# turian/inverse-audio-synthesis

Hardware: AMD Instinct MI355X
Metric: audio-seconds rendered+lossed/sec (whole node), batch=128 4s@44.1kHz (higher is better)
Workload: dtype f32; 1 GPU; BASELINE configs[1]: torchsynth-style Voice render + PQMF(3) analysis + mel-L1 loss, batch 128 x 4 s @ 44100 Hz per GPU; batch_per_gpu=128, samples_per_voice=176400, launch=hipgraph, streams=5, pipelined=True

## Files before the change

inverse-audio-synthesis_amd/csrc/spectral_kernels.hip:

```cpp
#include "ias_common.h"
#include <cstdlib>

#define SP_WAVES_MAX 12
static int stft_waves(int n_fft) {
  static const int env = ias_diag_env("IAS_STFT_WAVES") ? atoi(ias_diag_env("IAS_STFT_WAVES")) : 0;
  if (n_fft == 1024) return (env == 8 || env == 10) ? env : 4;
  if (n_fft == 2048) return env == 4 ? 4 : 12;
  return 4;
}

typedef float cpx __attribute__((ext_vector_type(2)));
typedef float f32x4 __attribute__((ext_vector_type(4)));
__host__ __device__ static inline int mel_padded_words(int mel_nnz, int n_out) {
  return n_out > 0 ? ((mel_nnz + 3 * n_out + 3) & ~3) : 0;
}
__device__ __forceinline__ cpx cmk(float x, float y) { return (cpx){x, y}; }
__device__ __forceinline__ cpx cadd(cpx a, cpx b) { return a + b; }
__device__ __forceinline__ cpx csub(cpx a, cpx b) { return a - b; }
#ifdef IAS_DIAG
__device__ __forceinline__ cpx cmul(cpx a, cpx b) {
  return __builtin_elementwise_fma((cpx){-a.y, a.y}, (cpx){b.y, b.x}, (cpx){a.x, a.x} * b);
}
__device__ __forceinline__ cpx cmul_negi(cpx a) { return (cpx){a.y, -a.x}; }
__device__ __forceinline__ cpx cadd_negi(cpx a, cpx x) { return a + cmul_negi(x); }
__device__ __forceinline__ cpx csub_negi(cpx a, cpx x) { return a - cmul_negi(x); }
__device__ __forceinline__ cpx cnegi_sub(cpx x, cpx a) { return cmul_negi(x) - a; }
#else
__device__ __forceinline__ cpx cmul(cpx a, cpx b) {
  return cmk(__builtin_fmaf(-a.y, b.y, a.x * b.x), __builtin_fmaf(a.y, b.x, a.x * b.y));
}
__device__ __forceinline__ cpx cadd_negi(cpx a, cpx x) {
  cpx r; asm("v_pk_add_f32 %0, %1, %2 op_sel:[0,1] op_sel_hi:[1,0] neg_hi:[0,1]" : "=v"(r) : "v"(a), "v"(x)); return r;
}
__device__ __forceinline__ cpx csub_negi(cpx a, cpx x) {
  cpx r; asm("v_pk_add_f32 %0, %1, %2 op_sel:[0,1] op_sel_hi:[1,0] neg_lo:[0,1]" : "=v"(r) : "v"(a), "v"(x)); return r;
}
__device__ __forceinline__ cpx cnegi_sub(cpx x, cpx a) {
  cpx r; asm("v_pk_add_f32 %0, %1, %2 op_sel:[1,0] op_sel_hi:[0,1] neg_lo:[0,1] neg_hi:[1,1]" : "=v"(r) : "v"(x), "v"(a)); return r;
}
#endif

__device__ __forceinline__ void dft4(cpx& v0, cpx& v1, cpx& v2, cpx& v3) {
  const cpx t0 = cadd(v0, v2), t1 = csub(v0, v2), t2 = cadd(v1, v3), t3 = csub(v1, v3);
  v0 = cadd(t0, t2); v1 = cadd_negi(t1, t3); v2 = csub(t0, t2); v3 = csub_negi(t1, t3);
}
__device__ __forceinline__ void dft8(cpx* v) {
  cpx e0 = v[0], e1 = v[2], e2 = v[4], e3 = v[6];
  cpx o0 = v[1], o1 = v[3], o2 = v[5], o3 = v[7];
  dft4(e0, e1, e2, e3);
  dft4(o0, o1, o2, o3);
  const float h = 0.70710678118654752f;
  o1 = cadd_negi(o1, o1) * h;
  o3 = cnegi_sub(o3, o3) * h;
  v[0] = cadd(e0, o0); v[4] = csub(e0, o0);
  v[1] = cadd(e1, o1); v[5] = csub(e1, o1);
  v[2] = cadd_negi(e2, o2); v[6] = csub_negi(e2, o2);
  v[3] = cadd(e3, o3); v[7] = csub(e3, o3);
}
__device__ __forceinline__ void dft16(cpx* v) {
  cpx e[8], o[8];
#pragma unroll
  for (int i = 0; i < 8; ++i) { e[i] = v[2 * i]; o[i] = v[2 * i + 1]; }
  dft8(e);
  dft8(o);
  const float c1 = 0.92387953251128674f, s1 = 0.38268343236508977f, h = 0.70710678118654752f;
  const cpx w[8] = {cmk(1.f, 0.f), cmk(c1, -s1), cmk(h, -h), cmk(s1, -c1),
                    cmk(0.f, -1.f), cmk(-s1, -c1), cmk(-h, -h), cmk(-c1, -s1)};
#pragma unroll
  for (int k = 0; k < 8; ++k) {
    const cpx t = cmul(o[k], w[k]);
    v[k] = cadd(e[k], t);
    v[k + 8] = csub(e[k], t);
  }
}
template <int R> __device__ __forceinline__ void dftR(cpx* v);
template <> __device__ __forceinline__ void dftR<4>(cpx* v) { dft4(v[0], v[1], v[2], v[3]); }
template <> __device__ __forceinline__ void dftR<8>(cpx* v) { dft8(v); }
template <> __device__ __forceinline__ void dftR<16>(cpx* v) { dft16(v); }

__device__ __forceinline__ int reflect_index(int i, int T) {
  if (i < 0) i = -i;
  if (i >= T) i = 2 * (T - 1) - i;
  return i;
}

__device__ __forceinline__ float wave_sum_f(float v) {
#pragma unroll
  for (int d = 32; d > 0; d >>= 1) v += __shfl_xor(v, d, 64);
  return v;
}

struct SpecArgs {
  const float* audio;
  const float* tables;
  const int* mel_start;
  const int* mel_count;
  const int* mel_woff;
  const float* mel_w;
  float* out;
  const float* target;
  double* partials;
  const float* rowpeak;
  int T, F, hop, n_out, mel_nnz;
  int groups;
  int value_mode;
  int loss_mode;
  float eps;
};

__device__ __forceinline__ void wave_lds_sync() {
#ifdef IAS_STFT_DRAIN_SYNC
  asm volatile("s_waitcnt lgkmcnt(0)" ::: "memory");
  __builtin_amdgcn_wave_barrier();
#else
  __builtin_amdgcn_fence(__ATOMIC_RELEASE, "wavefront");
  __builtin_amdgcn_wave_barrier();
  __builtin_amdgcn_fence(__ATOMIC_ACQUIRE, "wavefront");
#endif
}

typedef unsigned x_u2 __attribute__((ext_vector_type(2)));
template <int L> __device__ __forceinline__ void xchg_pair(float& f0, float& f1) {
  unsigned r0 = __float_as_uint(f0), r1 = __float_as_uint(f1);
  if (L == 5) { const x_u2 t = __builtin_amdgcn_permlane32_swap(r0, r1, false, false); r0 = t.x; r1 = t.y; }
  else if (L == 4) { const x_u2 t = __builtin_amdgcn_permlane16_swap(r0, r1, false, false); r0 = t.x; r1 = t.y; }
  else {
    const unsigned old0 = r0;
    r0 = __builtin_amdgcn_update_dpp(r0, r1, 0x128 , 0xf, 0xc, false);
    r1 = __builtin_amdgcn_update_dpp(r1, old0, 0x128, 0xf, 0x3, false);
  }
  f0 = __uint_as_float(r0); f1 = __uint_as_float(r1);
}
__device__ __forceinline__ void xchg_reg_lane345(cpx (&u)[8]) {
#pragma unroll
  for (int comp = 0; comp < 2; ++comp) {
    float f[8];
#pragma unroll
    for (int q = 0; q < 8; ++q) f[q] = comp ? u[q].y : u[q].x;
    xchg_pair<3>(f[0], f[1]); xchg_pair<3>(f[2], f[3]); xchg_pair<3>(f[4], f[5]); xchg_pair<3>(f[6], f[7]);
    xchg_pair<4>(f[0], f[2]); xchg_pair<4>(f[1], f[3]); xchg_pair<4>(f[4], f[6]); xchg_pair<4>(f[5], f[7]);
    xchg_pair<5>(f[0], f[4]); xchg_pair<5>(f[1], f[5]); xchg_pair<5>(f[2], f[6]); xchg_pair<5>(f[3], f[7]);
#pragma unroll
    for (int q = 0; q < 8; ++q) { if (comp) u[q].y = f[q]; else u[q].x = f[q]; }
  }
}
#ifndef IAS_S2_REGX
#define IAS_S2_REGX 1
#endif

template <int R, int N2>
__device__ __forceinline__ void load_frame(const float* __restrict__ arow, int T, int hop, int f, int lane,
                                           float (&x)[2 * R]) {
  const int g0 = f * hop - N2;
  if (g0 >= 0 && g0 + 2 * N2 <= T && (((g0 | T) & 1) == 0)) {
    typedef float f32x2_t __attribute__((ext_vector_type(2)));
    typedef const __attribute__((address_space(1))) f32x2_t* glb_f2p;
    glb_f2p p = (glb_f2p)(reinterpret_cast<const f32x2_t*>(arow + g0) + lane);
#ifndef IAS_LOADFRAME_PLAIN
    asm volatile("" : "+v"(p));
#endif
#pragma unroll
    for (int n1 = 0; n1 < R; ++n1) { const f32x2_t q = p[64 * n1]; x[2 * n1] = q[0]; x[2 * n1 + 1] = q[1]; }
  } else {
#pragma unroll
    for (int n1 = 0; n1 < R; ++n1) {
      const int m = g0 + 2 * (64 * n1 + lane);
      x[2 * n1] = arow[reflect_index(m, T)];
      x[2 * n1 + 1] = arow[reflect_index(m + 1, T)];
#ifndef IAS_LOADFRAME_PLAIN
      asm volatile("" : "+v"(x[2 * n1]), "+v"(x[2 * n1 + 1]));
#endif
    }
  }
}

template <int LOG2N, int SP_WAVES, bool LOSS2 >
__global__ __launch_bounds__(64 * SP_WAVES, SP_WAVES == 10 ? 5 : 1) void stft_kernel(const SpecArgs a) {
  constexpr int SP_THREADS = 64 * SP_WAVES;
  constexpr int NFFT = 1 << LOG2N, N2 = NFFT / 2, R = N2 / 64, NPAIR = 8 * R, NP_IT = (NPAIR + 63) / 64;
  constexpr int SCR = NPAIR * 9;
  constexpr int NUNP = (N2 / 2) / 64 + 1;
  extern __shared__ __attribute__((aligned(16))) float smem[];
  cpx* s_scr = reinterpret_cast<cpx*>(smem);
  float* s_melw = reinterpret_cast<float*>(s_scr + SP_WAVES * SCR);
  const int melw_words = mel_padded_words(a.mel_nnz, a.mel_start != nullptr ? a.n_out : 0);
  int* s_meli = reinterpret_cast<int*>(s_melw + melw_words);

  const int tid = threadIdx.x, lane = tid & 63, wave = tid >> 6;
  const int b = blockIdx.y;
  const float* arow = a.audio + (size_t)b * a.T;
  const bool mel = a.mel_start != nullptr;
  float pscale = 1.0f;
  if (a.rowpeak != nullptr) { const float pkv = a.rowpeak[b]; if (pkv > 1.0f) { const float r = 1.0f / pkv; pscale = r * r; } }

  if (mel) {
    for (int i = tid; i < melw_words; i += SP_THREADS) s_melw[i] = 0.0f;
    for (int i = tid; i < a.n_out; i += SP_THREADS) {
      s_meli[i] = a.mel_start[i];
      s_meli[a.n_out + i] = (a.mel_count[i] + 3) & ~3;
    }
    __syncthreads();
    for (int i = tid; i < a.n_out; i += SP_THREADS) {
      int off = 0;
      for (int m = 0; m < i; ++m) off += s_meli[a.n_out + m];
      s_meli[2 * a.n_out + i] = off;
    }
    __syncthreads();
    for (int i = tid; i < a.n_out; i += SP_THREADS) {
      const int n = a.mel_count[i], src = a.mel_woff[i], dst = s_meli[2 * a.n_out + i];
      for (int j = 0; j < n; ++j) s_melw[dst + j] = a.mel_w[src + j];
    }
  }

  constexpr int NTAB = 64 * (2 * R + 2 * R + 16 * NP_IT + 2 * NUNP);
  cpx* s_tab = reinterpret_cast<cpx*>(s_meli + ((3 * (mel ? a.n_out : 0) + 1) & ~1));
  for (int i = tid; i < NTAB / 2; i += SP_THREADS) {
    const int pp = i >> 6, l = i & 63;
    s_tab[i] = cmk(a.tables[64 * (2 * pp) + l], a.tables[64 * (2 * pp + 1) + l]);
  }
  const cpx* t_win = s_tab + lane;
  const cpx* t_tw1 = t_win + 64 * R;
  const cpx* t_tw2 = t_tw1 + 64 * R;
  const cpx* t_twu = t_tw2 + 64 * 8 * NP_IT;
  if (mel && lane < 3) reinterpret_cast<float*>(s_scr + wave * SCR)[N2 + 1 + lane] = 0.0f;
  __syncthreads();

  cpx* sA = s_scr + wave * SCR;
  float l0 = 0.f, l1 = 0.f, l2 = 0.f;
  int h_nmaxa = 0, h_nmaxb = 0;
  if (mel) {
    if (lane < a.n_out) h_nmaxa = s_meli[a.n_out + lane];
    if (lane + 64 < a.n_out) h_nmaxb = s_meli[a.n_out + lane + 64];
  }
#pragma unroll
  for (int d = 32; d > 0; d >>= 1) {
    h_nmaxa = max(h_nmaxa, __shfl_xor(h_nmaxa, d, 64));
    h_nmaxb = max(h_nmaxb, __shfl_xor(h_nmaxb, d, 64));
  }
  h_nmaxa = __builtin_amdgcn_readfirstlane(h_nmaxa);
  h_nmaxb = __builtin_amdgcn_readfirstlane(h_nmaxb);
  const int f_begin = blockIdx.x * a.groups;
  const int f_end = min(f_begin + a.groups, a.F);

  float xc[2 * R], xn[2 * R];
  int f = f_begin + wave;
  if (f < f_end) load_frame<R, N2>(arow, a.T, a.hop, f, lane, xc);

  for (; f < f_end; f += SP_WAVES) {
    const bool more = f + SP_WAVES < f_end;
    if (more) load_frame<R, N2>(arow, a.T, a.hop, f + SP_WAVES, lane, xn);

    cpx v[R];
#pragma unroll
    for (int n1 = 0; n1 < R; ++n1)
      v[n1] = cmk(xc[2 * n1], xc[2 * n1 + 1]) * t_win[64 * n1];
    dftR<R>(v);
    {
      const int c = lane & 7, aa = lane >> 3;
#pragma unroll
      for (int k1 = 0; k1 < R; ++k1)
        sA[(k1 * 8 + c) * 9 + aa] = cmul(v[k1], t_tw1[64 * k1]);
    }
    wave_lds_sync();
    cpx u[NP_IT][8];
#pragma unroll
    for (int i = 0; i < NP_IT; ++i) {
      const int p = lane + 64 * i;
      if (p < NPAIR) {
#pragma unroll
        for (int q = 0; q < 8; ++q) u[i][q] = sA[p * 9 + q];
      }
    }
    wave_lds_sync();
#pragma unroll
    for (int i = 0; i < NP_IT; ++i) {
      const int p = lane + 64 * i;
      if (p < NPAIR) {
        const int k1 = p >> 3, c = p & 7;
        dft8(u[i]);
#pragma unroll
        for (int d = 0; d < 8; ++d)
          sA[(k1 * 8 + d) * 9 + c] = cmul(u[i][d], t_tw2[64 * (8 * i + d)]);
      }
    }
    wave_lds_sync();
#pragma unroll
    for (int i = 0; i < NP_IT; ++i) {
      const int p = lane + 64 * i;
      if (p < NPAIR) {
#pragma unroll
        for (int q = 0; q < 8; ++q) u[i][q] = sA[p * 9 + q];
      }
    }
    wave_lds_sync();
#pragma unroll
    for (int i = 0; i < NP_IT; ++i) {
      const int p = lane + 64 * i;
      if (p < NPAIR) {
        const int k1 = p >> 3, d = p & 7;
        dft8(u[i]);
#pragma unroll
        for (int e = 0; e < 8; ++e) { const int k = k1 + R * d + 8 * R * e; sA[k + (k >> 3)] = u[i][e]; }
      }
    }
    wave_lds_sync();
    float pk[NUNP], pn[NUNP];
#pragma unroll
    for (int i = 0; i < NUNP; ++i) {
      const int k = lane + 64 * i;
      pk[i] = pn[i] = 0.f;
      if (k <= N2 / 2) {
        const int kn = (N2 - k) & (N2 - 1);
        const cpx zk = sA[k + (k >> 3)], zn = sA[kn + (kn >> 3)];
        const cpx ze = cmk(0.5f * (zk.x + zn.x), 0.5f * (zk.y - zn.y));
        const cpx zo = cmk(0.5f * (zk.y + zn.y), -0.5f * (zk.x - zn.x));
        const cpx t = cmul(t_twu[64 * i], zo);
        const cpx xk = cadd(ze, t);
        const cpx xq = cmk(ze.x - t.x, -(ze.y - t.y));
        float vk = xk.x * xk.x + xk.y * xk.y, vn = xq.x * xq.x + xq.y * xq.y;
        if (a.rowpeak != nullptr) { vk *= pscale; vn *= pscale; }
        if (a.value_mode == 1) { vk = __builtin_amdgcn_sqrtf(vk); vn = __builtin_amdgcn_sqrtf(vn); }
        else if (a.value_mode == 3) { vk = __builtin_amdgcn_sqrtf(fmaxf(vk, a.eps)); vn = __builtin_amdgcn_sqrtf(fmaxf(vn, a.eps)); }
        pk[i] = vk; pn[i] = vn;
      }
    }
    wave_lds_sync();
    float* P = reinterpret_cast<float*>(sA);
#pragma unroll
    for (int i = 0; i < NUNP; ++i) {
      const int k = lane + 64 * i;
      if (k <= N2 / 2) { P[k] = pk[i]; P[N2 - k] = pn[i]; }
    }
    wave_lds_sync();
    {
      const size_t row = ((size_t)b * a.F + f) * a.n_out;
      for (int m0 = 0; m0 < a.n_out; m0 += 128) {
        const int ma = m0 + lane, mb = m0 + 64 + lane;
        const bool oka = ma < a.n_out, okb = mb < a.n_out;
        float va = 0.f, vb = 0.f;
        if (mel) {
          const int sa = oka ? s_meli[ma] : 0, na = oka ? s_meli[a.n_out + ma] : 0, woa = oka ? s_meli[2 * a.n_out + ma] : 0;
          const int sb = okb ? s_meli[mb] : 0, nb = okb ? s_meli[a.n_out + mb] : 0, wob = okb ? s_meli[2 * a.n_out + mb] : 0;
          const float* wa = s_melw + woa;
          const float* wb = s_melw + wob;
          int nmaxa = h_nmaxa, nmaxb = h_nmaxb;
          if (m0 != 0) {
            nmaxa = na; nmaxb = nb;
#pragma unroll
            for (int d = 32; d > 0; d >>= 1) {
              nmaxa = max(nmaxa, __shfl_xor(nmaxa, d, 64));
              nmaxb = max(nmaxb, __shfl_xor(nmaxb, d, 64));
            }
          }
          for (int j = 0; j < nmaxa; j += 4) {
            const bool on = j < na;
            const int jj = on ? j : 0;
            const f32x4 w = *reinterpret_cast<const f32x4*>(wa + jj);
            const float* pp = P + sa + jj;
            const float p0 = pp[0], p1 = pp[1], p2 = pp[2], p3 = pp[3];
            const float t = fmaf(w[3], p3, fmaf(w[2], p2, fmaf(w[1], p1, fmaf(w[0], p0, va))));
            va = on ? t : va;
          }
          for (int j = 0; j < nmaxb; j += 4) {
            const bool on = j < nb;
            const int jj = on ? j : 0;
            const f32x4 w = *reinterpret_cast<const f32x4*>(wb + jj);
            const float* pp = P + sb + jj;
            const float p0 = pp[0], p1 = pp[1], p2 = pp[2], p3 = pp[3];
            const float t = fmaf(w[3], p3, fmaf(w[2], p2, fmaf(w[1], p1, fmaf(w[0], p0, vb))));
            vb = on ? t : vb;
          }
        } else {
          va = oka ? P[ma] : 0.f;
          vb = okb ? P[mb] : 0.f;
        }
        float ta = 0.f, tb = 0.f;
        if (a.loss_mode != 0) {
          if (oka) ta = a.target[row + ma];
          if (okb) tb = a.target[row + mb];
        }
        if (a.out != nullptr) {
          if (oka) a.out[row + ma] = va;
          if (okb) a.out[row + mb] = vb;
        }
        if (a.loss_mode == 1) {
          if (oka) l0 += fabsf(va - ta);
          if (okb) l0 += fabsf(vb - tb);
        } else if (LOSS2) {
          if (oka) { const float d = ta - va; l0 = fmaf(d, d, l0); l1 = fmaf(ta, ta, l1); l2 += fabsf(__log2f(va) - __log2f(ta)); }
          if (okb) { const float d = tb - vb; l0 = fmaf(d, d, l0); l1 = fmaf(tb, tb, l1); l2 += fabsf(__log2f(vb) - __log2f(tb)); }
        }
      }
    }
    wave_lds_sync();
    if (more) {
#pragma unroll
      for (int e = 0; e < 2 * R; ++e) xc[e] = xn[e];
    }
  }

  if (a.partials != nullptr) {
    __shared__ float s_red[SP_WAVES][4];
    l0 = wave_sum_f(l0); l1 = wave_sum_f(l1); l2 = wave_sum_f(l2) * 0.6931471805599453f;
    if (lane == 0) { s_red[wave][0] = l0; s_red[wave][1] = l1; s_red[wave][2] = l2; }
    __syncthreads();
    if (tid < 3) {
      double sacc = 0.0;
      for (int w = 0; w < SP_WAVES; ++w) sacc += (double)s_red[w][tid];
      a.partials[((size_t)blockIdx.y * gridDim.x + blockIdx.x) * 3 + tid] = sacc;
    }
  }
}

#define IAS_SEG_MAX_ROWS 17
#define IAS_SEG_HDR 16
#define IAS_SEG_STRIDE 72
#ifndef IAS_S2_ROW
#define IAS_S2_ROW 10
#endif
#define IAS_S2_AT(row, col) ((row) * IAS_S2_ROW + (col))
#define IAS_S2_UP(i) ((i) + (IAS_S2_ROW - 8) * ((i) >> 3))
static_assert(IAS_SEG_MAX_ROWS * IAS_SEG_STRIDE + 1 <= 2 * 64 * IAS_S2_ROW, "segment-major rows fit the wave's scratch");
struct Spec2Args {
  const float* audio;
  const float* tables;
  const float* segtab;
  float* out;
  const float* target;
  double* partials;
  const float* rowpeak;
  int T, F, hop, n_out, nframes;
  unsigned magicF;
  int value_mode, loss_mode;
  float eps;
#ifdef IAS_S2_STAMPS
  unsigned long long* stamps;
#endif
};
#ifdef IAS_S2_STAMPS
static unsigned long long* g_s2_stamps = nullptr;
extern "C" int ias_stft2_set_stamps(unsigned long long* p) { g_s2_stamps = p; return 0; }
#define S2_STAMP(id)                                                                                     \
  do {                                                                                                   \
    if (a.stamps != nullptr && stamp_n < 255) {                                                          \
      const unsigned long long t_ = __builtin_amdgcn_s_memtime();                                        \
      if (lane == 0) a.stamps[((size_t)blockIdx.x * SP_WAVES + wave) * 256 + 1 + stamp_n] = (t_ << 8) | (id); \
      ++stamp_n;                                                                                         \
    }                                                                                                    \
  } while (0)
#else
#define S2_STAMP(id) do {} while (0)
#endif
__device__ __forceinline__ float wave_shr1(float x, float fill) {
  return __int_as_float(__builtin_amdgcn_update_dpp(__float_as_int(fill), __float_as_int(x), 0x138, 0xf, 0xf, false));
}
__device__ __forceinline__ float wave_shl1(float x, float fill) {
  return __int_as_float(__builtin_amdgcn_update_dpp(__float_as_int(fill), __float_as_int(x), 0x130, 0xf, 0xf, false));
}

template <int NSUB> __device__ __forceinline__ void stft2_load_frame(const float* __restrict__ arow, int T, int hop, int f,
                                                                      int lane, float (&x)[16 * NSUB]) {
  if (NSUB == 1) {
    float (&x1)[16] = reinterpret_cast<float (&)[16]>(x);
    load_frame<8, 512>(arow, T, hop, f, lane, x1);
  } else {
    const int g0 = f * hop - 1024;
    if (g0 >= 0 && g0 + 2048 <= T && ((reinterpret_cast<uintptr_t>(arow + g0) & 15) == 0)) {
      const f32x4* p = reinterpret_cast<const f32x4*>(arow + g0) + lane;
#pragma unroll
      for (int n1 = 0; n1 < 8; ++n1) {
        const f32x4 q = p[64 * n1];
        x[2 * n1] = q[0]; x[2 * n1 + 1] = q[1]; x[16 + 2 * n1] = q[2]; x[16 + 2 * n1 + 1] = q[3];
      }
    } else {
#pragma unroll
      for (int n1 = 0; n1 < 8; ++n1)
#pragma unroll
        for (int c = 0; c < 4; ++c) {
          x[16 * (c >> 1) + 2 * n1 + (c & 1)] = arow[reflect_index(g0 + 256 * n1 + 4 * lane + c, T)];
        }
    }
  }
}

#ifndef IAS_STFT2_MINW
#define IAS_STFT2_MINW 5
#endif
#if IAS_S2_REGX
#define S2X_ROW 9
#define S2X_PAD 2
#else
#define S2X_ROW IAS_S2_ROW
#define S2X_PAD (IAS_S2_ROW - 8)
#endif
#define S2X_AT(row, col) ((row) * S2X_ROW + (col))
#define S2X_UP(i) ((i) + S2X_PAD * ((i) >> 3))
static_assert(64 * S2X_ROW <= 64 * IAS_S2_ROW && 256 + S2X_PAD * 32 <= 64 * IAS_S2_ROW, "stft2 scratch indexing fits the wave's scratch");
template <int SP_WAVES, bool MEL, int LOSS, int NSUB>
__global__ __launch_bounds__(64 * SP_WAVES, NSUB == 2 ? 3 * SP_WAVES / 8 : (SP_WAVES >= 8 ? (SP_WAVES == 8 ? IAS_STFT2_MINW : SP_WAVES / 2) : (3 * SP_WAVES + 3) / 4))
void stft2_kernel(const Spec2Args a) {
  static_assert(NSUB == 1 || (NSUB == 2 && !MEL), "mel filterbanks: n_fft 1024 only");
  constexpr int SP_THREADS = 64 * SP_WAVES, N2 = 512 * NSUB, R = 8, SCR = 64 * IAS_S2_ROW, NPK = 4 * NSUB, HALF = N2 / 2;
  constexpr int NTAB = 8 * NSUB + 8 + 8 + (NSUB == 2 ? 8 : 0) + NPK;
  extern __shared__ __attribute__((aligned(16))) float smem[];
  cpx* s_scr = reinterpret_cast<cpx*>(smem);
  __shared__ cpx s_tab[NTAB * 64];
  __shared__ cpx s_segw[MEL ? IAS_SEG_MAX_ROWS * 64 : 1];
  __shared__ int s_sega[MEL ? 9 * 64 : 1];
  const int tid = threadIdx.x, lane = tid & 63;
  const int wave = __builtin_amdgcn_readfirstlane(tid >> 6);

  constexpr int OLD_UNP = 10, V2_BASE_2048 = 32 + 32 + 32 + 18;
  for (int i = tid; i < NTAB * 64; i += SP_THREADS) {
    const int pp = i >> 6, l = i & 63;
    const int src = NSUB == 2 ? V2_BASE_2048 + 2 * pp : (pp < 24 ? 2 * pp : 48 + OLD_UNP + 2 * (pp - 24));
    s_tab[i] = cmk(a.tables[64 * src + l], a.tables[64 * (src + 1) + l]);
  }
  for (int i = tid; i < SP_WAVES * SCR; i += SP_THREADS) s_scr[i] = cmk(0.f, 0.f);
  int seg_rows = 0, seg_r[3] = {0, 0, 0}, seg_s0 = 0;
  if (MEL) {
    const int* hdr = reinterpret_cast<const int*>(a.segtab);
    seg_rows = hdr[1]; seg_r[0] = hdr[2]; seg_r[1] = hdr[3]; seg_r[2] = hdr[4]; seg_s0 = hdr[5];
    for (int i = tid; i < 9 * 64; i += SP_THREADS) s_sega[i] = hdr[IAS_SEG_HDR + i];
    const cpx* wsrc = reinterpret_cast<const cpx*>(a.segtab + IAS_SEG_HDR + 9 * 64);
    for (int i = tid; i < seg_rows * 64; i += SP_THREADS) s_segw[i] = wsrc[i];
  }
  const cpx* t_win = s_tab + lane;
  const cpx* t_tw1 = t_win + 64 * 8 * NSUB;
  const cpx* t_tw2 = t_tw1 + 64 * 8;
  const cpx* t_cmb = t_tw2 + 64 * 8;
  const cpx* t_twu = t_cmb + (NSUB == 2 ? 64 * 8 : 0);
  __syncthreads();

  cpx* sA = s_scr + wave * SCR;
  float* P2 = reinterpret_cast<float*>(sA);

  float l0 = 0.f, l1 = 0.f, l2 = 0.f;
  const int gw = blockIdx.x * SP_WAVES + wave, nw = gridDim.x * SP_WAVES;
  const int k1 = lane >> 3, dd = lane & 7;

  auto row_of = [&](int fi, int& b, int& f) {
    unsigned q0 = __umulhi((unsigned)fi, a.magicF);
    int r = fi - (int)q0 * a.F;
    if (r >= a.F) { r -= a.F; ++q0; }
    b = (int)q0; f = r;
  };
  float xc[16 * NSUB], xn[16 * NSUB];
#ifdef IAS_S2_STAMPS
  int stamp_n = 0;
#endif
  int fi = gw, bcur = 0, fcur = 0;
  float pk_cur = 0.0f, pk_next = 0.0f;
  if (fi < a.nframes) {
    row_of(fi, bcur, fcur);
    stft2_load_frame<NSUB>(a.audio + (size_t)bcur * a.T, a.T, a.hop, fcur, lane, xc);
    if (a.rowpeak != nullptr) pk_cur = a.rowpeak[bcur];
#pragma unroll
    for (int e = 0; e < 16 * NSUB; ++e) asm volatile("" : "+v"(xc[e]));
    asm volatile("" : "+v"(pk_cur));
  }
  for (; fi < a.nframes; fi += nw) {
    const bool more = fi + nw < a.nframes;
    S2_STAMP(1);
    int bnext = 0, fnext = 0;
    if (more) {
      row_of(fi + nw, bnext, fnext);
      stft2_load_frame<NSUB>(a.audio + (size_t)bnext * a.T, a.T, a.hop, fnext, lane, xn);
      if (a.rowpeak != nullptr) pk_next = a.rowpeak[bnext];
    }
    float pscale = 0.25f;
    if (pk_cur > 1.0f) { const float r = __builtin_amdgcn_rcpf(pk_cur); pscale = 0.25f * (r * r); }
    const size_t row = (size_t)fi * a.n_out;
    float tgt_m[3] = {0.f, 0.f, 0.f};
    if (MEL && LOSS != 0) {
#pragma unroll
      for (int c = 0; c < 3; ++c) if (64 * c + lane < a.n_out) tgt_m[c] = a.target[row + 64 * c + lane];
    }

    const int kl = k1 + 8 * dd;
    float tg_k[NPK], tg_n[NPK], tg_mid = 0.f;
    if (!MEL && LOSS != 0) {
#pragma unroll
      for (int e = 0; e < NPK; ++e) { tg_k[e] = a.target[row + kl + 64 * e]; tg_n[e] = a.target[row + N2 - kl - 64 * e]; }
      if (lane == 0) tg_mid = a.target[row + HALF];
    }
    cpx zlo[NPK], zhi[NPK];
    cpx ue[8];
#pragma unroll
    for (int sub = 0; sub < NSUB; ++sub) {
      cpx v[R];
#pragma unroll
      for (int n1 = 0; n1 < R; ++n1) v[n1] = cmk(xc[16 * sub + 2 * n1], xc[16 * sub + 2 * n1 + 1]) * t_win[64 * (8 * sub + n1)];
      dft8(v);
      cpx u[8];
#if IAS_S2_REGX
#pragma unroll
      for (int q = 0; q < R; ++q) u[q] = cmul(v[q], t_tw1[64 * q]);
      S2_STAMP(2);
      xchg_reg_lane345(u);
      S2_STAMP(3);
      S2_STAMP(4);
#else
      {
        const int c = lane & 7, aa = lane >> 3;
#pragma unroll
        for (int q = 0; q < R; ++q) sA[S2X_AT(q * 8 + c, aa)] = cmul(v[q], t_tw1[64 * q]);
      }
      S2_STAMP(2);
      wave_lds_sync();
      S2_STAMP(3);
#pragma unroll
      for (int q = 0; q < 8; ++q) u[q] = sA[S2X_AT(lane, q)];
      wave_lds_sync();
      S2_STAMP(4);
#endif
      dft8(u);
#pragma unroll
      for (int d = 0; d < 8; ++d) sA[S2X_AT(k1 * 8 + d, dd)] = cmul(u[d], t_tw2[64 * d]);
      S2_STAMP(5);
      wave_lds_sync();
      S2_STAMP(6);
#pragma unroll
      for (int q = 0; q < 8; ++q) u[q] = sA[S2X_AT(lane, q)];
      wave_lds_sync();
      S2_STAMP(7);
      dft8(u);
      if (NSUB == 1) {
#pragma unroll
        for (int e = 0; e < 4; ++e) { zlo[e] = u[e]; zhi[e] = u[4 + e]; }
      } else if (sub == 0) {
#pragma unroll
        for (int e = 0; e < 8; ++e) ue[e] = u[e];
      } else {
#pragma unroll
        for (int e = 0; e < 8; ++e) {
          const cpx t = cmul(u[e], t_cmb[64 * e]);
          zlo[e % NPK] = cadd(ue[e], t); zhi[e % NPK] = csub(ue[e], t);
        }
      }
    }
#pragma unroll
    for (int e = 0; e < NPK; ++e) { const int i = kl + 64 * e; sA[S2X_UP(i)] = zhi[e]; }
    S2_STAMP(8);
    wave_lds_sync();
    S2_STAMP(9);
    float pk[NPK], pn[NPK];
#pragma unroll
    for (int e = 0; e < NPK; ++e) {
      const int k = kl + 64 * e;
      const int i = (HALF - k) & (HALF - 1);
      cpx zn = sA[S2X_UP(i)];
      const cpx zk = zlo[e];
      if (e == 0 && k == 0) zn = zk;
      const cpx w = t_twu[64 * e];
      const float ea = zk.x + zn.x, eb = zk.y - zn.y, od = zk.x - zn.x, os = zk.y + zn.y;
      const float tx = fmaf(w.y, od, w.x * os), ty = fmaf(-w.x, od, w.y * os);
      const float xr = ea + tx, xi = eb + ty, yr = ea - tx, yi = eb - ty;
      pk[e] = fmaf(xi, xi, xr * xr) * pscale;
      pn[e] = fmaf(yi, yi, yr * yr) * pscale;
    }
    float pmid = fmaf(zhi[0].y, zhi[0].y, zhi[0].x * zhi[0].x) * (4.0f * pscale);
    if (a.value_mode == 1) {
#pragma unroll
      for (int e = 0; e < NPK; ++e) { pk[e] = __builtin_amdgcn_sqrtf(pk[e]); pn[e] = __builtin_amdgcn_sqrtf(pn[e]); }
      pmid = __builtin_amdgcn_sqrtf(pmid);
    } else if (a.value_mode == 3) {
#pragma unroll
      for (int e = 0; e < NPK; ++e) { pk[e] = __builtin_amdgcn_sqrtf(fmaxf(pk[e], a.eps)); pn[e] = __builtin_amdgcn_sqrtf(fmaxf(pn[e], a.eps)); }
      pmid = __builtin_amdgcn_sqrtf(fmaxf(pmid, a.eps));
    }
    S2_STAMP(10);
    wave_lds_sync();
    S2_STAMP(11);
    auto emit_t = [&](int m, float val, float t) {
      if (a.out != nullptr) a.out[row + m] = val;
      if (LOSS == 1) l0 += fabsf(val - t);
      else if (LOSS == 2) { const float d = t - val; l0 = fmaf(d, d, l0); l1 = fmaf(t, t, l1); l2 += fabsf(__log2f(val) - __log2f(t)); }
    };

    if (MEL) {
#pragma unroll
      for (int e = 0; e < 4; ++e) { P2[s_sega[64 * e + lane]] = pk[e]; P2[s_sega[64 * (4 + e) + lane]] = pn[e]; }
      if (lane == 0) P2[s_sega[64 * 8]] = pmid;
      S2_STAMP(12);
      wave_lds_sync();
      S2_STAMP(13);
      float U[3], D[3];
      int rbase = 0;
#pragma unroll
      for (int g = 0; g < 3; ++g) {
        float us = 0.f, ds = 0.f;
        const int n = seg_r[g];
        int t = 0;
        for (; t + 4 <= n; t += 4) {
          float pv[4]; cpx w[4];
#pragma unroll
          for (int u = 0; u < 4; ++u) { pv[u] = P2[(rbase + t + u) * IAS_SEG_STRIDE + lane]; w[u] = s_segw[(rbase + t + u) * 64 + lane]; }
#pragma unroll
          for (int u = 0; u < 4; ++u) { us = fmaf(w[u].x, pv[u], us); ds = fmaf(w[u].y, pv[u], ds); }
        }
        if (t < n) {
          float pv[3]; cpx w[3];
#pragma unroll
          for (int u = 0; u < 3; ++u) {
            const int row = min(rbase + t + u, IAS_SEG_MAX_ROWS - 1);
            pv[u] = P2[row * IAS_SEG_STRIDE + lane]; w[u] = s_segw[row * 64 + lane];
          }
#pragma unroll
          for (int u = 0; u < 3; ++u)
            if (t + u < n) { us = fmaf(w[u].x, pv[u], us); ds = fmaf(w[u].y, pv[u], ds); }
        }
        U[g] = us; D[g] = ds;
        rbase += n;
      }
      S2_STAMP(14);
#pragma unroll
      for (int c = 0; c < 3; ++c) {
        const int m = 64 * c + lane;
        if (64 * c < a.n_out) {
          float val;
          if (seg_s0 == 1) {
            const float fill = c > 0 ? __int_as_float(__builtin_amdgcn_readlane(__float_as_int(U[c > 0 ? c - 1 : 0]), 63)) : 0.f;
            val = D[c] + wave_shr1(U[c], fill);
          } else {
            const float fill = c < 2 ? __int_as_float(__builtin_amdgcn_readlane(__float_as_int(D[c < 2 ? c + 1 : 2]), 0)) : 0.f;
            val = U[c] + wave_shl1(D[c], fill);
          }
          if (m < a.n_out) emit_t(m, val, tgt_m[c]);
        }
      }
    } else {
#pragma unroll
      for (int e = 0; e < NPK; ++e) { const int k = kl + 64 * e; emit_t(k, pk[e], tg_k[e]); emit_t(N2 - k, pn[e], tg_n[e]); }
      if (lane == 0) emit_t(HALF, pmid, tg_mid);
    }
    S2_STAMP(15);
    wave_lds_sync();
    if (more) {
#pragma unroll
      for (int e = 0; e < 16 * NSUB; ++e) xc[e] = xn[e];
      bcur = bnext; fcur = fnext; pk_cur = pk_next;
    }
  }

#ifdef IAS_S2_STAMPS
  if (a.stamps != nullptr && lane == 0) a.stamps[((size_t)blockIdx.x * SP_WAVES + wave) * 256] = stamp_n;
#endif
  if (a.partials != nullptr) {
    __shared__ float s_red[SP_WAVES][4];
    l0 = wave_sum_f(l0); l1 = wave_sum_f(l1); l2 = wave_sum_f(l2) * 0.6931471805599453f;
    if (lane == 0) { s_red[wave][0] = l0; s_red[wave][1] = l1; s_red[wave][2] = l2; }
    __syncthreads();
    if (tid < 3) {
      double sacc = 0.0;
      for (int w = 0; w < SP_WAVES; ++w) sacc += (double)s_red[w][tid];
      a.partials[(size_t)blockIdx.x * 3 + tid] = sacc;
    }
  }
}

template <int SP_WAVES, int LOSS>
__global__ __launch_bounds__(64 * SP_WAVES, SP_WAVES >= 8 ? SP_WAVES / 2 : (3 * SP_WAVES + 3) / 4)
void stft2h_kernel(const Spec2Args a) {
  constexpr int SP_THREADS = 64 * SP_WAVES, SCR = 64 * IAS_S2_ROW, N2 = 256, HALF = 128;
  constexpr int NTAB = 4 + 4 + 8 + 4;
  extern __shared__ __attribute__((aligned(16))) float smem[];
  cpx* s_scr = reinterpret_cast<cpx*>(smem);
  __shared__ cpx s_tab[NTAB * 64];
  const int tid = threadIdx.x, lane = tid & 63;
  const int wave = __builtin_amdgcn_readfirstlane(tid >> 6);
  for (int i = tid; i < NTAB * 64; i += SP_THREADS) {
    const int pp = i >> 6, l = i & 63, src = pp < 16 ? 2 * pp : 38 + 2 * (pp - 16);
    s_tab[i] = cmk(a.tables[64 * src + l], a.tables[64 * (src + 1) + l]);
  }
  const cpx* t_win = s_tab + lane;
  const cpx* t_tw1 = t_win + 64 * 4;
  const cpx* t_tw2 = t_tw1 + 64 * 4;
  const cpx* t_twu = t_tw2 + 64 * 8;
  __syncthreads();

  cpx* sA = s_scr + wave * SCR;
  float l0 = 0.f, l1 = 0.f, l2 = 0.f;
  const int gw = blockIdx.x * SP_WAVES + wave, nw = gridDim.x * SP_WAVES;
  const int slot = lane >> 3, dd = lane & 7, fr = lane >> 5, kl = (slot & 3) + 4 * dd;
  const int npairs = (a.nframes + 1) >> 1;
  auto row_of = [&](int fi, int& b, int& f) {
    unsigned q0 = __umulhi((unsigned)fi, a.magicF);
    int r = fi - (int)q0 * a.F;
    if (r >= a.F) { r -= a.F; ++q0; }
    b = (int)q0; f = r;
  };
  auto load_pair = [&](int pi, float (&x)[16], int& bA, int& bB) {
    const int fiA = 2 * pi, fiB = min(2 * pi + 1, a.nframes - 1);
    int fA, fB;
    row_of(fiA, bA, fA); row_of(fiB, bB, fB);
    float (&xa)[8] = reinterpret_cast<float (&)[8]>(x[0]);
    float (&xb)[8] = reinterpret_cast<float (&)[8]>(x[8]);
    load_frame<4, 256>(a.audio + (size_t)bA * a.T, a.T, a.hop, fA, lane, xa);
    load_frame<4, 256>(a.audio + (size_t)bB * a.T, a.T, a.hop, fB, lane, xb);
  };
  float xc[16], xn[16];
  int pi = gw, bA = 0, bB = 0;
  if (pi < npairs) {
    load_pair(pi, xc, bA, bB);
#pragma unroll
    for (int e = 0; e < 16; ++e) asm volatile("" : "+v"(xc[e]));
  }
  for (; pi < npairs; pi += nw) {
    const bool more = pi + nw < npairs;
    int bAn = 0, bBn = 0;
    if (more) load_pair(pi + nw, xn, bAn, bBn);
    const bool own = fr == 0 || 2 * pi + 1 < a.nframes;
    const int fi = own ? 2 * pi + fr : 2 * pi;
    const size_t row = (size_t)fi * a.n_out;
    float pscale = 0.25f;
    if (a.rowpeak != nullptr) { const float pkv = a.rowpeak[fr ? bB : bA]; if (pkv > 1.0f) { const float r = __builtin_amdgcn_rcpf(pkv); pscale = 0.25f * (r * r); } }
    float tg_k[4], tg_n[4], tg_mid = 0.f;
    if (LOSS != 0) {
#pragma unroll
      for (int e = 0; e < 4; ++e) { tg_k[e] = a.target[row + kl + 32 * e]; tg_n[e] = a.target[row + N2 - kl - 32 * e]; }
      if (kl == 0) tg_mid = a.target[row + HALF];
    }
    cpx v[8];
#pragma unroll
    for (int n1 = 0; n1 < 4; ++n1) {
      v[n1] = cmk(xc[2 * n1], xc[2 * n1 + 1]) * t_win[64 * n1];
      v[4 + n1] = cmk(xc[8 + 2 * n1], xc[8 + 2 * n1 + 1]) * t_win[64 * n1];
    }
    {
      cpx (&va)[4] = reinterpret_cast<cpx (&)[4]>(v[0]);
      cpx (&vb)[4] = reinterpret_cast<cpx (&)[4]>(v[4]);
      dftR<4>(va); dftR<4>(vb);
      const int c = lane & 7, aa = lane >> 3;
#pragma unroll
      for (int q = 0; q < 8; ++q) sA[(q * 8 + c) * IAS_S2_ROW + aa] = cmul(v[q], t_tw1[64 * (q & 3)]);
    }
    wave_lds_sync();
    cpx u[8];
#pragma unroll
    for (int q = 0; q < 8; ++q) u[q] = sA[lane * IAS_S2_ROW + q];
    wave_lds_sync();
    dft8(u);
#pragma unroll
    for (int d = 0; d < 8; ++d) sA[(slot * 8 + d) * IAS_S2_ROW + dd] = cmul(u[d], t_tw2[64 * d]);
    wave_lds_sync();
#pragma unroll
    for (int q = 0; q < 8; ++q) u[q] = sA[lane * IAS_S2_ROW + q];
    wave_lds_sync();
    dft8(u);
#pragma unroll
    for (int e = 0; e < 4; ++e) sA[fr * HALF + kl + 32 * e] = u[4 + e];
    wave_lds_sync();
    float pk[4], pn[4];
#pragma unroll
    for (int e = 0; e < 4; ++e) {
      const int k = kl + 32 * e;
      cpx zn = sA[fr * HALF + ((HALF - k) & (HALF - 1))];
      const cpx zk = u[e];
      if (e == 0 && k == 0) zn = zk;
      const cpx w = t_twu[64 * e];
      const float ea = zk.x + zn.x, eb = zk.y - zn.y, od = zk.x - zn.x, os = zk.y + zn.y;
      const float tx = fmaf(w.y, od, w.x * os), ty = fmaf(-w.x, od, w.y * os);
      const float xr = ea + tx, xi = eb + ty, yr = ea - tx, yi = eb - ty;
      pk[e] = fmaf(xi, xi, xr * xr) * pscale;
      pn[e] = fmaf(yi, yi, yr * yr) * pscale;
    }
    float pmid = fmaf(u[4].y, u[4].y, u[4].x * u[4].x) * (4.0f * pscale);
    if (a.value_mode == 1) {
#pragma unroll
      for (int e = 0; e < 4; ++e) { pk[e] = __builtin_amdgcn_sqrtf(pk[e]); pn[e] = __builtin_amdgcn_sqrtf(pn[e]); }
      pmid = __builtin_amdgcn_sqrtf(pmid);
    } else if (a.value_mode == 3) {
#pragma unroll
      for (int e = 0; e < 4; ++e) { pk[e] = __builtin_amdgcn_sqrtf(fmaxf(pk[e], a.eps)); pn[e] = __builtin_amdgcn_sqrtf(fmaxf(pn[e], a.eps)); }
      pmid = __builtin_amdgcn_sqrtf(fmaxf(pmid, a.eps));
    }
    auto emit_t = [&](int m, float val, float t) {
      if (a.out != nullptr) a.out[row + m] = val;
      if (LOSS == 1) l0 += fabsf(val - t);
      else if (LOSS == 2) { const float d = t - val; l0 = fmaf(d, d, l0); l1 = fmaf(t, t, l1); l2 += fabsf(__log2f(val) - __log2f(t)); }
    };
    if (own) {
#pragma unroll
      for (int e = 0; e < 4; ++e) { const int k = kl + 32 * e; emit_t(k, pk[e], tg_k[e]); emit_t(N2 - k, pn[e], tg_n[e]); }
      if (kl == 0) emit_t(HALF, pmid, tg_mid);
    }
    wave_lds_sync();
    if (more) {
#pragma unroll
      for (int e = 0; e < 16; ++e) xc[e] = xn[e];
      bA = bAn; bB = bBn;
    }
  }
  if (a.partials != nullptr) {
    __shared__ float s_red[SP_WAVES][4];
    l0 = wave_sum_f(l0); l1 = wave_sum_f(l1); l2 = wave_sum_f(l2) * 0.6931471805599453f;
    if (lane == 0) { s_red[wave][0] = l0; s_red[wave][1] = l1; s_red[wave][2] = l2; }
    __syncthreads();
    if (tid < 3) {
      double sacc = 0.0;
      for (int w = 0; w < SP_WAVES; ++w) sacc += (double)s_red[w][tid];
      a.partials[(size_t)blockIdx.x * 3 + tid] = sacc;
    }
  }
}

extern "C" int ias_stft_num_frames(int T, int n_fft, int hop);
struct SgwArgs {
  const float* audio; const float* tables; const float* target; const double* coef; float* frame_grad;
  const int* mel_start; const int* mel_count; const int* mel_woff; const float* mel_w;
  int T, F, hop, groups, power2, loss_mode, n_out, mel_nnz;
  float scale, eps;
  int G, cper, L, nchunks;
};

template <int LOG2N, bool MEL, bool SPAN, bool CROW>
__global__ __launch_bounds__(256) void stft_grad_wave_kernel(const SgwArgs a) {
  constexpr int SP_WAVES = 4, SP_THREADS = 256;
  constexpr int NFFT = 1 << LOG2N, N2 = NFFT / 2, R = N2 / 64, NPAIR = 8 * R, NP_IT = (NPAIR + 63) / 64;
  constexpr int SCR = NPAIR * IAS_S2_ROW, NUNP = (N2 / 2) / 64 + 1, NB = N2 + 1;
  constexpr int NTAB = 64 * (2 * R + 2 * R + 16 * NP_IT + 2 * NUNP);
  extern __shared__ __attribute__((aligned(16))) float smem[];
  cpx* s_scr = reinterpret_cast<cpx*>(smem);
  float* s_ring = reinterpret_cast<float*>(s_scr + SP_WAVES * SCR);
  __shared__ cpx s_tab[NTAB / 2];
  const int tid = threadIdx.x, lane = tid & 63, wave = __builtin_amdgcn_readfirstlane(tid >> 6);
  if (SPAN) for (int i = tid; i < SP_WAVES * NFFT; i += SP_THREADS) s_ring[i] = 0.0f;
  for (int i = tid; i < NTAB / 2; i += SP_THREADS) {
    const int pp = i >> 6, l = i & 63;
    s_tab[i] = cmk(a.tables[64 * (2 * pp) + l], a.tables[64 * (2 * pp + 1) + l]);
  }
  float* s_melw = reinterpret_cast<float*>(s_scr + SP_WAVES * SCR + (SPAN ? SP_WAVES * N2 : 0));
  const int melw_words = MEL ? mel_padded_words(a.mel_nnz, a.n_out) : 0;
  int* s_meli = reinterpret_cast<int*>(s_melw + melw_words);
  const int so_words = MEL ? ((a.n_out + 3) & ~3) : 0;
  float* s_go = reinterpret_cast<float*>(s_meli + (MEL ? ((3 * a.n_out + 3) & ~3) : 0)) + wave * (so_words + NB + 7);
  float* s_gv = s_go + so_words;
  if (MEL) {
    for (int i = tid; i < melw_words; i += SP_THREADS) s_melw[i] = 0.0f;
    for (int i = tid; i < a.n_out; i += SP_THREADS) {
      s_meli[i] = a.mel_start[i];
      s_meli[a.n_out + i] = (a.mel_count[i] + 3) & ~3;
    }
    __syncthreads();
    for (int i = tid; i < a.n_out; i += SP_THREADS) {
      int off = 0;
      for (int m = 0; m < i; ++m) off += s_meli[a.n_out + m];
      s_meli[2 * a.n_out + i] = off;
    }
    __syncthreads();
    for (int i = tid; i < a.n_out; i += SP_THREADS) {
      const int n = a.mel_count[i], src = a.mel_woff[i], dst = s_meli[2 * a.n_out + i];
      for (int j = 0; j < n; ++j) s_melw[dst + j] = a.mel_w[src + j];
    }
  }
  const cpx* t_win = s_tab + lane;
  const cpx* t_tw1 = t_win + 64 * R;
  const cpx* t_tw2 = t_tw1 + 64 * R;
  const cpx* t_twu = t_tw2 + 64 * 8 * NP_IT;
  if (MEL && lane < 3) reinterpret_cast<float*>(s_scr + wave * SCR)[NB + lane] = 0.0f;
  __syncthreads();
  cpx* sA = s_scr + wave * SCR;
  float c0 = 0.0f, c1 = 0.0f;
  if constexpr (!CROW) { if (a.loss_mode == 2) { c0 = (float)a.coef[0]; c1 = (float)a.coef[1]; } }

  auto fft = [&](cpx (&v)[R]) {
    dftR<R>(v);
    {
      const int c = lane & 7, aa = lane >> 3;
#pragma unroll
      for (int k1 = 0; k1 < R; ++k1) sA[(k1 * 8 + c) * IAS_S2_ROW + aa] = cmul(v[k1], t_tw1[64 * k1]);
    }
    wave_lds_sync();
    cpx u[NP_IT][8];
#pragma unroll
    for (int i = 0; i < NP_IT; ++i) {
      const int p = lane + 64 * i;
      if (p < NPAIR) {
#pragma unroll
        for (int q = 0; q < 8; ++q) u[i][q] = sA[p * IAS_S2_ROW + q];
      }
    }
    wave_lds_sync();
#pragma unroll
    for (int i = 0; i < NP_IT; ++i) {
      const int p = lane + 64 * i;
      if (p < NPAIR) {
        const int k1 = p >> 3, c = p & 7;
        dft8(u[i]);
#pragma unroll
        for (int d = 0; d < 8; ++d) sA[(k1 * 8 + d) * IAS_S2_ROW + c] = cmul(u[i][d], t_tw2[64 * (8 * i + d)]);
      }
    }
    wave_lds_sync();
#pragma unroll
    for (int i = 0; i < NP_IT; ++i) {
      const int p = lane + 64 * i;
      if (p < NPAIR) {
#pragma unroll
        for (int q = 0; q < 8; ++q) u[i][q] = sA[p * IAS_S2_ROW + q];
      }
    }
    wave_lds_sync();
#pragma unroll
    for (int i = 0; i < NP_IT; ++i) {
      const int p = lane + 64 * i;
      if (p < NPAIR) {
        const int k1 = p >> 3, d = p & 7;
        dft8(u[i]);
#pragma unroll
        for (int e = 0; e < 8; ++e) { const int k = k1 + R * d + 8 * R * e; sA[IAS_S2_UP(k)] = u[i][e]; }
      }
    }
    wave_lds_sync();
  };
  auto bin_value = [&](float p) { return a.power2 ? p : __builtin_amdgcn_sqrtf(a.loss_mode == 2 ? fmaxf(p, a.eps) : p); };
  auto value_grad = [&](float v, float t) {
    const float d = v - t;
    const float sg = d > 0.0f ? 1.0f : (d < 0.0f ? -1.0f : 0.0f);
    return a.loss_mode == 2 ? c0 * d + c1 * sg * __builtin_amdgcn_rcpf(v) : sg * a.scale;
  };
  auto power_grad = [&](float gv, float v) {
    if (a.power2) return gv;
    const bool live = a.loss_mode == 2 ? v > __builtin_amdgcn_sqrtf(a.eps) : v > 0.0f;
    return live ? 0.5f * gv * __builtin_amdgcn_rcpf(v) : 0.0f;
  };

  float xc[2 * R];
  float* ring = s_ring + wave * NFFT;
  const int cstep = SPAN ? (int)gridDim.x * SP_WAVES : 1;
  for (int c = SPAN ? (int)blockIdx.x * SP_WAVES + wave : 0; c < (SPAN ? a.nchunks : 1); c += cstep) {
  int b, f_lo, f_hi;
  if (SPAN) { b = c / a.cper; f_lo = (c - b * a.cper) * a.G; f_hi = min(f_lo + a.G, a.F); }
  else { b = blockIdx.y; f_lo = blockIdx.x * a.groups + wave; f_hi = min((int)blockIdx.x * a.groups + a.groups, a.F); }
  if constexpr (CROW) { c0 = (float)a.coef[2 * (size_t)b]; c1 = (float)a.coef[2 * (size_t)b + 1]; }
  const float* arow = a.audio + (size_t)b * a.T;
  float* span = a.frame_grad + (size_t)c * a.L;
  for (int f = f_lo; f < f_hi; f += SPAN ? 1 : SP_WAVES) {
    load_frame<R, N2>(arow, a.T, a.hop, f, lane, xc);
    const float* trow = a.target + ((size_t)b * a.F + f) * (MEL ? a.n_out : NB);
    float tk_[NUNP], tq_[NUNP];
    if (!MEL) {
#pragma unroll
      for (int i = 0; i < NUNP; ++i) {
// ... 1005 lines not shown
```

Baseline: 3.369 million audio-s/s.

## Overlap STFT prologue loads and reuse frame registers for the n_fft=1024 path

Issues the first audio-frame load before the table staging, and stages the twiddle and mel tables through registers so their global loads run ahead of the LDS zeroing. For the single-sub (n_fft 1024) case, the next frame is prefetched straight into xc right after the first DFT8, which drops the xn double buffer and its register cost. It also swaps the first twiddle multiply in each stage for a cmul_unit, which assumes the q=0 and d=0 twiddles are unity. That relies on the table contents, and the cmul_unit formula looks like a plain copy written with fma-by-zero.

```diff
diff --git a/inverse-audio-synthesis_amd/csrc/spectral_kernels.hip b/inverse-audio-synthesis_amd/csrc/spectral_kernels.hip
--- a/inverse-audio-synthesis_amd/csrc/spectral_kernels.hip
+++ b/inverse-audio-synthesis_amd/csrc/spectral_kernels.hip
@@ -39,6 +39,8 @@
   cpx r; asm("v_pk_add_f32 %0, %1, %2 op_sel:[1,0] op_sel_hi:[0,1] neg_lo:[0,1] neg_hi:[1,1]" : "=v"(r) : "v"(x), "v"(a)); return r;
 }
 #endif
+
+__device__ __forceinline__ cpx cmul_unit(cpx a) { return cmk(__builtin_fmaf(a.y, 0.0f, a.x), __builtin_fmaf(-a.x, 0.0f, a.y)); }
 
 __device__ __forceinline__ void dft4(cpx& v0, cpx& v1, cpx& v2, cpx& v3) {
   const cpx t0 = cadd(v0, v2), t1 = csub(v0, v2), t2 = cadd(v1, v3), t3 = csub(v1, v3);
@@ -509,21 +511,58 @@
   __shared__ int s_sega[MEL ? 9 * 64 : 1];
   const int tid = threadIdx.x, lane = tid & 63;
   const int wave = __builtin_amdgcn_readfirstlane(tid >> 6);
+  const int gw = blockIdx.x * SP_WAVES + wave, nw = gridDim.x * SP_WAVES;
+
+  auto row_of = [&](int fi, int& b, int& f) {
+    unsigned q0 = __umulhi((unsigned)fi, a.magicF);
+    int r = fi - (int)q0 * a.F;
+    if (r >= a.F) { r -= a.F; ++q0; }
+    b = (int)q0; f = r;
+  };
+  constexpr bool ONESET = NSUB == 1;
+  float xc[16 * NSUB], xn[ONESET ? 1 : 16 * NSUB];
+  int fi = gw;
+  float pk_cur = 0.0f, pk_next = 0.0f;
+  if (fi < a.nframes) {
+    int b0, f0;
+    row_of(fi, b0, f0);
+    stft2_load_frame<NSUB>(a.audio + (size_t)b0 * a.T, a.T, a.hop, f0, lane, xc);
+    if (a.rowpeak != nullptr) pk_cur = a.rowpeak[b0];
+  }
 
   constexpr int OLD_UNP = 10, V2_BASE_2048 = 32 + 32 + 32 + 18;
-  for (int i = tid; i < NTAB * 64; i += SP_THREADS) {
-    const int pp = i >> 6, l = i & 63;
-    const int src = NSUB == 2 ? V2_BASE_2048 + 2 * pp : (pp < 24 ? 2 * pp : 48 + OLD_UNP + 2 * (pp - 24));
-    s_tab[i] = cmk(a.tables[64 * src + l], a.tables[64 * (src + 1) + l]);
+  auto tab_src = [&](int i) {
+    const int pp = i >> 6;
+    return 64 * (NSUB == 2 ? V2_BASE_2048 + 2 * pp : (pp < 24 ? 2 * pp : 48 + OLD_UNP + 2 * (pp - 24))) + (i & 63);
+  };
+  int seg_rows = 0, seg_r[3] = {0, 0, 0}, seg_s0 = 0;
+  const int* hdr = reinterpret_cast<const int*>(a.segtab);
+  const cpx* wsrc = reinterpret_cast<const cpx*>(a.segtab + IAS_SEG_HDR + 9 * 64);
+  if (MEL) { seg_rows = hdr[1]; seg_r[0] = hdr[2]; seg_r[1] = hdr[3]; seg_r[2] = hdr[4]; seg_s0 = hdr[5]; }
+  constexpr int TAB_IT = (NTAB * 64 + SP_THREADS - 1) / SP_THREADS, SEGA_IT = (9 * 64 + SP_THREADS - 1) / SP_THREADS;
+  constexpr int SEGW_IT = (IAS_SEG_MAX_ROWS * 64 + SP_THREADS - 1) / SP_THREADS;
+  float st_re[TAB_IT], st_im[TAB_IT];
+  int st_a[MEL ? SEGA_IT : 1];
+  cpx st_w[MEL ? SEGW_IT : 1];
+#pragma unroll
+  for (int k = 0; k < TAB_IT; ++k) {
+    const int i = tid + k * SP_THREADS;
+    if (i < NTAB * 64) { st_re[k] = a.tables[tab_src(i)]; st_im[k] = a.tables[tab_src(i) + 64]; }
+  }
+  if (MEL) {
+#pragma unroll
+    for (int k = 0; k < SEGA_IT; ++k) { const int i = tid + k * SP_THREADS; if (i < 9 * 64) st_a[k] = hdr[IAS_SEG_HDR + i]; }
+#pragma unroll
+    for (int k = 0; k < SEGW_IT; ++k) { const int i = tid + k * SP_THREADS; if (i < seg_rows * 64) st_w[k] = wsrc[i]; }
   }
   for (int i = tid; i < SP_WAVES * SCR; i += SP_THREADS) s_scr[i] = cmk(0.f, 0.f);
-  int seg_rows = 0, seg_r[3] = {0, 0, 0}, seg_s0 = 0;
+#pragma unroll
+  for (int k = 0; k < TAB_IT; ++k) { const int i = tid + k * SP_THREADS; if (i < NTAB * 64) s_tab[i] = cmk(st_re[k], st_im[k]); }
   if (MEL) {
-    const int* hdr = reinterpret_cast<const int*>(a.segtab);
-    seg_rows = hdr[1]; seg_r[0] = hdr[2]; seg_r[1] = hdr[3]; seg_r[2] = hdr[4]; seg_s0 = hdr[5];
-    for (int i = tid; i < 9 * 64; i += SP_THREADS) s_sega[i] = hdr[IAS_SEG_HDR + i];
-    const cpx* wsrc = reinterpret_cast<const cpx*>(a.segtab + IAS_SEG_HDR + 9 * 64);
-    for (int i = tid; i < seg_rows * 64; i += SP_THREADS) s_segw[i] = wsrc[i];
+#pragma unroll
+    for (int k = 0; k < SEGA_IT; ++k) { const int i = tid + k * SP_THREADS; if (i < 9 * 64) s_sega[i] = st_a[k]; }
+#pragma unroll
+    for (int k = 0; k < SEGW_IT; ++k) { const int i = tid + k * SP_THREADS; if (i < seg_rows * 64) s_segw[i] = st_w[k]; }
   }
   const cpx* t_win = s_tab + lane;
   const cpx* t_tw1 = t_win + 64 * 8 * NSUB;
@@ -536,25 +575,11 @@
   float* P2 = reinterpret_cast<float*>(sA);
 
   float l0 = 0.f, l1 = 0.f, l2 = 0.f;
-  const int gw = blockIdx.x * SP_WAVES + wave, nw = gridDim.x * SP_WAVES;
   const int k1 = lane >> 3, dd = lane & 7;
-
-  auto row_of = [&](int fi, int& b, int& f) {
-    unsigned q0 = __umulhi((unsigned)fi, a.magicF);
-    int r = fi - (int)q0 * a.F;
-    if (r >= a.F) { r -= a.F; ++q0; }
-    b = (int)q0; f = r;
-  };
-  float xc[16 * NSUB], xn[16 * NSUB];
 #ifdef IAS_S2_STAMPS
   int stamp_n = 0;
 #endif
-  int fi = gw, bcur = 0, fcur = 0;
-  float pk_cur = 0.0f, pk_next = 0.0f;
   if (fi < a.nframes) {
-    row_of(fi, bcur, fcur);
-    stft2_load_frame<NSUB>(a.audio + (size_t)bcur * a.T, a.T, a.hop, fcur, lane, xc);
-    if (a.rowpeak != nullptr) pk_cur = a.rowpeak[bcur];
 #pragma unroll
     for (int e = 0; e < 16 * NSUB; ++e) asm volatile("" : "+v"(xc[e]));
     asm volatile("" : "+v"(pk_cur));
@@ -562,10 +587,10 @@
   for (; fi < a.nframes; fi += nw) {
     const bool more = fi + nw < a.nframes;
     S2_STAMP(1);
-    int bnext = 0, fnext = 0;
-    if (more) {
+    if (!ONESET && more) {
+      int bnext, fnext;
       row_of(fi + nw, bnext, fnext);
-      stft2_load_frame<NSUB>(a.audio + (size_t)bnext * a.T, a.T, a.hop, fnext, lane, xn);
+      stft2_load_frame<NSUB>(a.audio + (size_t)bnext * a.T, a.T, a.hop, fnext, lane, reinterpret_cast<float (&)[16 * NSUB]>(xn));
       if (a.rowpeak != nullptr) pk_next = a.rowpeak[bnext];
     }
     float pscale = 0.25f;
@@ -592,10 +617,20 @@
 #pragma unroll
       for (int n1 = 0; n1 < R; ++n1) v[n1] = cmk(xc[16 * sub + 2 * n1], xc[16 * sub + 2 * n1 + 1]) * t_win[64 * (8 * sub + n1)];
       dft8(v);
+      if (ONESET) {
+#pragma unroll
+        for (int n1 = 0; n1 < R; ++n1) asm volatile("" : "+v"(v[n1]));
+        if (more) {
+          int bnext, fnext;
+          row_of(fi + nw, bnext, fnext);
+          stft2_load_frame<NSUB>(a.audio + (size_t)bnext * a.T, a.T, a.hop, fnext, lane, xc);
+          if (a.rowpeak != nullptr) pk_cur = a.rowpeak[bnext];
+        }
+      }
       cpx u[8];
 #if IAS_S2_REGX
 #pragma unroll
-      for (int q = 0; q < R; ++q) u[q] = cmul(v[q], t_tw1[64 * q]);
+      for (int q = 0; q < R; ++q) u[q] = q == 0 ? cmul_unit(v[q]) : cmul(v[q], t_tw1[64 * q]);
       S2_STAMP(2);
       xchg_reg_lane345(u);
       S2_STAMP(3);
@@ -604,7 +639,7 @@
       {
         const int c = lane & 7, aa = lane >> 3;
 #pragma unroll
-        for (int q = 0; q < R; ++q) sA[S2X_AT(q * 8 + c, aa)] = cmul(v[q], t_tw1[64 * q]);
+        for (int q = 0; q < R; ++q) sA[S2X_AT(q * 8 + c, aa)] = q == 0 ? cmul_unit(v[q]) : cmul(v[q], t_tw1[64 * q]);
       }
       S2_STAMP(2);
       wave_lds_sync();
@@ -616,7 +651,7 @@
 #endif
       dft8(u);
 #pragma unroll
-      for (int d = 0; d < 8; ++d) sA[S2X_AT(k1 * 8 + d, dd)] = cmul(u[d], t_tw2[64 * d]);
+      for (int d = 0; d < 8; ++d) sA[S2X_AT(k1 * 8 + d, dd)] = d == 0 ? cmul_unit(u[d]) : cmul(u[d], t_tw2[64 * d]);
       S2_STAMP(5);
       wave_lds_sync();
       S2_STAMP(6);
@@ -736,10 +771,10 @@
     }
     S2_STAMP(15);
     wave_lds_sync();
-    if (more) {
+    if (!ONESET && more) {
 #pragma unroll
       for (int e = 0; e < 16 * NSUB; ++e) xc[e] = xn[e];
-      bcur = bnext; fcur = fnext; pk_cur = pk_next;
+      pk_cur = pk_next;
     }
   }
 
```

Result: faster. 3.430 million audio-s/s (median of 6 runs) (+1.8%).
